# IDEA-Research/MP-Former

Measured on AMD Instinct MI355X. Metric: training images/sec COCO-instance R50 1024x1024, higher is better.
Workload: dtype bf16 (backbone, decoder) + f32 (pixel decoder, losses), as the reference's AMP; 1 GPU; COCO-instance R50, 100 queries, 80 classes, 1024x1024: full train step = R50 backbone + MSDeformAttn pixel decoder (6 layers) + MP masked decoder (9 layers, NUM_DN 1) + Hungarian matching + 60 losses + backward + grad all-reduce + clip + AdamW; head_only_workload=False, global_batch=2, per_gpu_batch=2, parallelism=dp1, msda_offsets=init, full=False, autograd_threads=backward on the launch thread, miopen_find_db=shipped

## Files before the change

mp_former_amd/csrc/gemm3_nt2.h:

```cpp
constexpr int kN2T = 512;
constexpr int kN2Kc = 256 * 16;
constexpr int kN2Op = 2 * 4 * kN2Kc;
constexpr int kN2Stage = 2 * kN2Op;
constexpr int kN2Lds = 2 * kN2Stage;

struct AccN2 {
    f32x16 v[4][2];
    __device__ __forceinline__ void zero()
    {
#pragma unroll
        for (int i = 0; i < 4; ++i)
#pragma unroll
            for (int j = 0; j < 2; ++j)
#pragma unroll
                for (int e = 0; e < 16; ++e) v[i][j][e] = 0.f;
    }
    __device__ __forceinline__ void step(const unsigned char* st, int a_base, int b_base, int lane)
    {
        const int r32 = lane & 31, gh = lane >> 5;
#pragma unroll
        for (int kh = 0; kh < 2; ++kh) {
            const int kc = 2 * kh + gh;
            const int sw = (r32 ^ (2 * kc)) * 16;
            f16x8 fb[2][2];
#pragma unroll
            for (int pl = 0; pl < 2; ++pl)
#pragma unroll
                for (int t = 0; t < 2; ++t) fb[pl][t] = as_fragh(*reinterpret_cast<const uint4*>(st + kN2Op + b_base + (pl * 4 + kc) * kN2Kc + t * 512 + sw));
#pragma unroll
            for (int i = 0; i < 4; ++i) {
                const f16x8 fah = as_fragh(*reinterpret_cast<const uint4*>(st + a_base + (0 * 4 + kc) * kN2Kc + i * 512 + sw));
                const f16x8 fal = as_fragh(*reinterpret_cast<const uint4*>(st + a_base + (1 * 4 + kc) * kN2Kc + i * 512 + sw));
#pragma unroll
                for (int j = 0; j < 2; ++j) v[i][j] = __builtin_amdgcn_mfma_f32_32x32x16_f16(fb[1][j], fah, v[i][j], 0, 0, 0);
#pragma unroll
                for (int j = 0; j < 2; ++j) v[i][j] = __builtin_amdgcn_mfma_f32_32x32x16_f16(fb[0][j], fal, v[i][j], 0, 0, 0);
#pragma unroll
                for (int j = 0; j < 2; ++j) v[i][j] = __builtin_amdgcn_mfma_f32_32x32x16_f16(fb[0][j], fah, v[i][j], 0, 0, 0);
            }
        }
    }
};

template <bool CV>
__device__ __forceinline__ void gemm3_nt2_tile(const G3N& p, const int tile, unsigned char* lds)
{
    float sc_a, sc_b, inv_a, inv_b;
    h2_scale(amax_read(p.a_amax), &sc_a, &inv_a);
    h2_scale(amax_read(p.b_amax), &sc_b, &inv_b);
    const int tn = tile % p.tiles_n, tm = (tile / p.tiles_n) % p.tiles_m, sp = tile / (p.tiles_n * p.tiles_m);
    const int m0 = tm * 256, n0 = tn * 256;
    const int r_begin = sp * p.rows_per_split, r_end = min(p.R, r_begin + p.rows_per_split);
    const int tid = threadIdx.x, lane = tid & 63, wave = tid >> 6;
    const int wr = wave >> 2, wc = wave & 3;

    const int col = tid & 255, kc0 = __builtin_amdgcn_readfirstlane(tid >> 8);
    const __amdgpu_buffer_rsrc_t ars = __builtin_amdgcn_make_buffer_rsrc(const_cast<float*>(p.a), 0, p.a_bytes, 0x00020000);
    const __amdgpu_buffer_rsrc_t brs = __builtin_amdgcn_make_buffer_rsrc(const_cast<float*>(p.b), 0, p.b_bytes, 0x00020000);
    const int acolb = (m0 + col) * 4, bcolb = (CV ? (n0 % p.cv_cin) + col : n0 + col) * 4;
    const int ldab = (int)p.lda * 4, ldbb = (int)p.ldb * 4;
    int cv_dy = 0, cv_dx = 0, cv_sh = 0, cvx0 = 0, cvy0 = 0, cvx1 = 0, cvy1 = 0;
    if constexpr (CV) {
        const int tap = n0 / p.cv_cin;
        cv_dy = tap / 3 - 1; cv_dx = tap % 3 - 1;
        cv_sh = cv_dy * p.cv_W + cv_dx;
        const int rb0 = r_begin + kc0 * 8, rb1 = rb0 + 16;
        cvx0 = rb0 % p.cv_W; cvy0 = (rb0 / p.cv_W) % p.cv_H;
        cvx1 = rb1 % p.cv_W; cvy1 = (rb1 / p.cv_W) % p.cv_H;
    }
    (void)cv_dy; (void)cv_dx; (void)cv_sh;
    float xa0[8], xa1[8], xb0[8], xb1[8];
    float csa = 0.f;
    const bool want_csa = p.csum_a && tn == 0;

#define N2_LOAD_A(r0, TAIL)                                                                                      \
    {                                                                                                            \
        _Pragma("unroll") for (int j = 0; j < 8; ++j) {                                                          \
            const int q0 = (r0) + kc0 * 8 + j, q1 = q0 + 16;                                                     \
            const int c0 = TAIL ? min(q0, r_end - 1) : q0, c1 = TAIL ? min(q1, r_end - 1) : q1;                  \
            float va0 = __int_as_float(__builtin_amdgcn_raw_buffer_load_b32(ars, acolb, c0 * ldab, 0));          \
            float va1 = __int_as_float(__builtin_amdgcn_raw_buffer_load_b32(ars, acolb, c1 * ldab, 0));          \
            if (TAIL) { va0 = q0 < r_end ? va0 : 0.f; va1 = q1 < r_end ? va1 : 0.f; }                            \
            xa0[j] = va0; xa1[j] = va1;                                                                          \
        }                                                                                                        \
    }
#define N2_LOAD_B(r0, TAIL)                                                                                      \
    {                                                                                                            \
        _Pragma("unroll") for (int j = 0; j < 8; ++j) {                                                          \
            const int q0 = (r0) + kc0 * 8 + j, q1 = q0 + 16;                                                     \
            int c0 = TAIL ? min(q0, r_end - 1) : q0, c1 = TAIL ? min(q1, r_end - 1) : q1;                        \
            if constexpr (CV) { c0 = min(max(c0 + cv_sh, 0), p.R - 1); c1 = min(max(c1 + cv_sh, 0), p.R - 1); }  \
            float vb0 = __int_as_float(__builtin_amdgcn_raw_buffer_load_b32(brs, bcolb, c0 * ldbb, 0));          \
            float vb1 = __int_as_float(__builtin_amdgcn_raw_buffer_load_b32(brs, bcolb, c1 * ldbb, 0));          \
            if constexpr (CV) {                                                                                  \
                const bool ok0 = (unsigned)(cvy0 + cv_dy) < (unsigned)p.cv_H && (unsigned)(cvx0 + j + cv_dx) < (unsigned)p.cv_W; \
                const bool ok1 = (unsigned)(cvy1 + cv_dy) < (unsigned)p.cv_H && (unsigned)(cvx1 + j + cv_dx) < (unsigned)p.cv_W; \
                vb0 = ok0 ? vb0 : 0.f; vb1 = ok1 ? vb1 : 0.f;                                                    \
            }                                                                                                    \
            if (TAIL) { vb0 = q0 < r_end ? vb0 : 0.f; vb1 = q1 < r_end ? vb1 : 0.f; }                            \
            xb0[j] = vb0; xb1[j] = vb1;                                                                          \
        }                                                                                                        \
        if constexpr (CV) {                                              \
            cvx0 += kBK; while (cvx0 >= p.cv_W) { cvx0 -= p.cv_W; cvy0 = cvy0 + 1 == p.cv_H ? 0 : cvy0 + 1; }    \
            cvx1 += kBK; while (cvx1 >= p.cv_W) { cvx1 -= p.cv_W; cvy1 = cvy1 + 1 == p.cv_H ? 0 : cvy1 + 1; }    \
        }                                                                                                        \
    }
#define N2_LOAD(r0, TAIL) { N2_LOAD_A(r0, TAIL) N2_LOAD_B(r0, TAIL) }

    AccN2 acc;
    acc.zero();
    const int a_base = wr * 128 * 16, b_base = wc * 64 * 16;
    const int sl0 = (col ^ (2 * kc0)) * 16, sl1 = (col ^ (2 * kc0 + 4)) * 16;

    if (r_begin + kBK <= r_end) N2_LOAD(r_begin, false) else N2_LOAD(r_begin, true);
    int s = 0;
    for (int r0 = r_begin; r0 < r_end; r0 += kBK, s ^= 1) {
        unsigned char* st = lds + s * kN2Stage;
        uint4 h, l;
        const bool full_next = r0 + 2 * kBK <= r_end, some_next = r0 + kBK < r_end;
        split8h(make_float4(xa0[0], xa0[1], xa0[2], xa0[3]), make_float4(xa0[4], xa0[5], xa0[6], xa0[7]), sc_a, &h, &l);
        *reinterpret_cast<uint4*>(st + (0 * 4 + kc0) * kN2Kc + sl0) = h;
        *reinterpret_cast<uint4*>(st + (1 * 4 + kc0) * kN2Kc + sl0) = l;
        split8h(make_float4(xa1[0], xa1[1], xa1[2], xa1[3]), make_float4(xa1[4], xa1[5], xa1[6], xa1[7]), sc_a, &h, &l);
        *reinterpret_cast<uint4*>(st + (0 * 4 + kc0 + 2) * kN2Kc + sl1) = h;
        *reinterpret_cast<uint4*>(st + (1 * 4 + kc0 + 2) * kN2Kc + sl1) = l;
        if (want_csa) {
#pragma unroll
            for (int j = 0; j < 8; ++j) csa += xa0[j] + xa1[j];
        }
        if (full_next) N2_LOAD_A(r0 + kBK, false) else if (some_next) N2_LOAD_A(r0 + kBK, true);
        split8h(make_float4(xb0[0], xb0[1], xb0[2], xb0[3]), make_float4(xb0[4], xb0[5], xb0[6], xb0[7]), sc_b, &h, &l);
        *reinterpret_cast<uint4*>(st + kN2Op + (0 * 4 + kc0) * kN2Kc + sl0) = h;
        *reinterpret_cast<uint4*>(st + kN2Op + (1 * 4 + kc0) * kN2Kc + sl0) = l;
        split8h(make_float4(xb1[0], xb1[1], xb1[2], xb1[3]), make_float4(xb1[4], xb1[5], xb1[6], xb1[7]), sc_b, &h, &l);
        *reinterpret_cast<uint4*>(st + kN2Op + (0 * 4 + kc0 + 2) * kN2Kc + sl1) = h;
        *reinterpret_cast<uint4*>(st + kN2Op + (1 * 4 + kc0 + 2) * kN2Kc + sl1) = l;
        if (full_next) N2_LOAD_B(r0 + kBK, false) else if (some_next) N2_LOAD_B(r0 + kBK, true);
        ws_barrier();
        acc.step(st, a_base, b_base, lane);
    }
#undef N2_LOAD
#undef N2_LOAD_A
#undef N2_LOAD_B

    float* cp = p.c + (int64_t)sp * p.c_ss;
    {
        const int r32 = lane & 31, gh = lane >> 5;
#pragma unroll
        for (int j = 0; j < 2; ++j)
#pragma unroll
            for (int i = 0; i < 4; ++i)
#pragma unroll
                for (int q = 0; q < 4; ++q) {
                    const int m = m0 + wr * 128 + i * 32 + r32, n = n0 + wc * 64 + j * 32 + 8 * q + 4 * gh;
                    float4 o = make_float4(acc.v[i][j][4 * q], acc.v[i][j][4 * q + 1], acc.v[i][j][4 * q + 2], acc.v[i][j][4 * q + 3]);
                    o = make_float4(o.x * inv_a * inv_b, o.y * inv_a * inv_b, o.z * inv_a * inv_b, o.w * inv_a * inv_b);
                    *reinterpret_cast<float4*>(cp + (int64_t)m * p.Ndim + n) = o;
                }
    }
    if (want_csa) {
        __syncthreads();
        float* red = reinterpret_cast<float*>(lds);
        if (tid < 256) red[tid] = csa;
        __syncthreads();
        if (tid >= 256) red[col] += csa;
        __syncthreads();
        if (tid < 256) p.csum_a[(int64_t)sp * p.csa_ss + m0 + tid] = red[tid];
    }
}

__global__ __launch_bounds__(kN2T, 2) void gemm3_nt2_group_kernel(G3NG g)
{
    extern __shared__ __attribute__((aligned(16))) unsigned char n2_lds[];
    const int per_xcd = (g.ntiles + 7) >> 3;
    const int tile = ((int)blockIdx.x & 7) * per_xcd + ((int)blockIdx.x >> 3);
    if (tile >= g.ntiles) return;
    int i = 0;
    while (i + 1 < g.n_items && tile >= g.tile_end[i]) ++i;
    const int first = i ? g.tile_end[i - 1] : 0;
    gemm3_nt2_tile<false>(g.it[i], tile - first, n2_lds);
}

__global__ __launch_bounds__(kN2T, 2) void gemm3_nt2_conv_kernel(G3N p)
{
    extern __shared__ __attribute__((aligned(16))) unsigned char n2_lds[];
    const int per_xcd = (p.ntiles + 7) >> 3;
    const int tile = ((int)blockIdx.x & 7) * per_xcd + ((int)blockIdx.x >> 3);
    if (tile >= p.ntiles) return;
    gemm3_nt2_tile<true>(p, tile, n2_lds);
}
```

Before: 87.42 images/sec.

## Software-pipeline the split-f16 GEMM main loop by interleaving MFMAs with staging and loads

Restructures the gemm3_nt2 main loop into a prologue plus a steady-state body. Each MFMA pair is interleaved with fine-grained split-to-f16 conversion, LDS stores into the next buffer and global loads for the stage after that, with one barrier per iteration. The A/B fragments are prefetched from LDS ahead of their MFMAs, and the conv-mode bounds check becomes a bitmask that is applied later. The goal is to hide global-load and conversion latency behind tensor-core work. It adds register pressure and more complex control flow, and sched_barriers pin the instruction order.

Result: no change. 86.97 images/sec (-0.5%).

```diff
diff --git a/mp_former_amd/csrc/gemm3_nt2.h b/mp_former_amd/csrc/gemm3_nt2.h
--- a/mp_former_amd/csrc/gemm3_nt2.h
+++ b/mp_former_amd/csrc/gemm3_nt2.h
@@ -4,6 +4,17 @@
 constexpr int kN2Stage = 2 * kN2Op;
 constexpr int kN2Lds = 2 * kN2Stage;
 
+__device__ __forceinline__ void split2h(const float x0, const float x1, const float scale, unsigned* h, unsigned* l)
+{
+    const float s0 = x0 * scale, s1 = x1 * scale;
+    const f16x2 hh = {(_Float16)s0, (_Float16)s1};
+    const float r0 = s0 - (float)hh[0], r1 = s1 - (float)hh[1];
+    const f16x2 ll = {(_Float16)r0, (_Float16)r1};
+    union { f16x2 f; unsigned u; } ch, cl;
+    ch.f = hh; cl.f = ll;
+    *h = ch.u; *l = cl.u;
+}
+
 struct AccN2 {
     f32x16 v[4][2];
     __device__ __forceinline__ void zero()
@@ -15,28 +26,39 @@
 #pragma unroll
                 for (int e = 0; e < 16; ++e) v[i][j][e] = 0.f;
     }
+    static __device__ __forceinline__ int frag_off(int lane, int kh, int pl)
+    {
+        const int kc = 2 * kh + (lane >> 5);
+        return (pl * 4 + kc) * kN2Kc + ((lane & 31) ^ (2 * kc)) * 16;
+    }
+    static __device__ __forceinline__ f16x8 frag_b(const unsigned char* st, int b_base, int lane, int kh, int pl, int t)
+    {
+        return as_fragh(*reinterpret_cast<const uint4*>(st + kN2Op + b_base + frag_off(lane, kh, pl) + t * 512));
+    }
+    static __device__ __forceinline__ f16x8 frag_a(const unsigned char* st, int a_base, int lane, int kh, int pl, int i)
+    {
+        return as_fragh(*reinterpret_cast<const uint4*>(st + a_base + frag_off(lane, kh, pl) + i * 512));
+    }
+    __device__ __forceinline__ void pair(int i, const f16x8 (&fb)[2], const f16x8& fa)
+    {
+#pragma unroll
+        for (int j = 0; j < 2; ++j) v[i][j] = __builtin_amdgcn_mfma_f32_32x32x16_f16(fb[j], fa, v[i][j], 0, 0, 0);
+    }
     __device__ __forceinline__ void step(const unsigned char* st, int a_base, int b_base, int lane)
     {
-        const int r32 = lane & 31, gh = lane >> 5;
 #pragma unroll
         for (int kh = 0; kh < 2; ++kh) {
-            const int kc = 2 * kh + gh;
-            const int sw = (r32 ^ (2 * kc)) * 16;
             f16x8 fb[2][2];
 #pragma unroll
             for (int pl = 0; pl < 2; ++pl)
 #pragma unroll
-                for (int t = 0; t < 2; ++t) fb[pl][t] = as_fragh(*reinterpret_cast<const uint4*>(st + kN2Op + b_base + (pl * 4 + kc) * kN2Kc + t * 512 + sw));
+                for (int t = 0; t < 2; ++t) fb[pl][t] = frag_b(st, b_base, lane, kh, pl, t);
 #pragma unroll
             for (int i = 0; i < 4; ++i) {
-                const f16x8 fah = as_fragh(*reinterpret_cast<const uint4*>(st + a_base + (0 * 4 + kc) * kN2Kc + i * 512 + sw));
-                const f16x8 fal = as_fragh(*reinterpret_cast<const uint4*>(st + a_base + (1 * 4 + kc) * kN2Kc + i * 512 + sw));
-#pragma unroll
-                for (int j = 0; j < 2; ++j) v[i][j] = __builtin_amdgcn_mfma_f32_32x32x16_f16(fb[1][j], fah, v[i][j], 0, 0, 0);
-#pragma unroll
-                for (int j = 0; j < 2; ++j) v[i][j] = __builtin_amdgcn_mfma_f32_32x32x16_f16(fb[0][j], fal, v[i][j], 0, 0, 0);
-#pragma unroll
-                for (int j = 0; j < 2; ++j) v[i][j] = __builtin_amdgcn_mfma_f32_32x32x16_f16(fb[0][j], fah, v[i][j], 0, 0, 0);
+                const f16x8 fah = frag_a(st, a_base, lane, kh, 0, i), fal = frag_a(st, a_base, lane, kh, 1, i);
+                pair(i, fb[1], fah);
+                pair(i, fb[0], fal);
+                pair(i, fb[0], fah);
             }
         }
     }
@@ -59,7 +81,7 @@
     const __amdgpu_buffer_rsrc_t brs = __builtin_amdgcn_make_buffer_rsrc(const_cast<float*>(p.b), 0, p.b_bytes, 0x00020000);
     const int acolb = (m0 + col) * 4, bcolb = (CV ? (n0 % p.cv_cin) + col : n0 + col) * 4;
     const int ldab = (int)p.lda * 4, ldbb = (int)p.ldb * 4;
-    int cv_dy = 0, cv_dx = 0, cv_sh = 0, cvx0 = 0, cvy0 = 0, cvx1 = 0, cvy1 = 0;
+    int cv_dy = 0, cv_dx = 0, cv_sh = 0, cvx0 = 0, cvy0 = 0, cvx1 = 0, cvy1 = 0, cv_sx = 0, cv_sy = 0;
     if constexpr (CV) {
         const int tap = n0 / p.cv_cin;
         cv_dy = tap / 3 - 1; cv_dx = tap % 3 - 1;
@@ -67,79 +89,148 @@
         const int rb0 = r_begin + kc0 * 8, rb1 = rb0 + 16;
         cvx0 = rb0 % p.cv_W; cvy0 = (rb0 / p.cv_W) % p.cv_H;
         cvx1 = rb1 % p.cv_W; cvy1 = (rb1 / p.cv_W) % p.cv_H;
-    }
-    (void)cv_dy; (void)cv_dx; (void)cv_sh;
+        cv_sx = kBK % p.cv_W; cv_sy = (kBK / p.cv_W) % p.cv_H;
+    }
+    (void)cv_dy; (void)cv_dx; (void)cv_sh; (void)cv_sx; (void)cv_sy;
     float xa0[8], xa1[8], xb0[8], xb1[8];
     float csa = 0.f;
+    unsigned cv_ok = 0;
+    (void)cv_ok;
     const bool want_csa = p.csum_a && tn == 0;
 
-#define N2_LOAD_A(r0, TAIL)                                                                                      \
-    {                                                                                                            \
-        _Pragma("unroll") for (int j = 0; j < 8; ++j) {                                                          \
-            const int q0 = (r0) + kc0 * 8 + j, q1 = q0 + 16;                                                     \
-            const int c0 = TAIL ? min(q0, r_end - 1) : q0, c1 = TAIL ? min(q1, r_end - 1) : q1;                  \
-            float va0 = __int_as_float(__builtin_amdgcn_raw_buffer_load_b32(ars, acolb, c0 * ldab, 0));          \
-            float va1 = __int_as_float(__builtin_amdgcn_raw_buffer_load_b32(ars, acolb, c1 * ldab, 0));          \
-            if (TAIL) { va0 = q0 < r_end ? va0 : 0.f; va1 = q1 < r_end ? va1 : 0.f; }                            \
-            xa0[j] = va0; xa1[j] = va1;                                                                          \
-        }                                                                                                        \
-    }
-#define N2_LOAD_B(r0, TAIL)                                                                                      \
-    {                                                                                                            \
-        _Pragma("unroll") for (int j = 0; j < 8; ++j) {                                                          \
-            const int q0 = (r0) + kc0 * 8 + j, q1 = q0 + 16;                                                     \
-            int c0 = TAIL ? min(q0, r_end - 1) : q0, c1 = TAIL ? min(q1, r_end - 1) : q1;                        \
-            if constexpr (CV) { c0 = min(max(c0 + cv_sh, 0), p.R - 1); c1 = min(max(c1 + cv_sh, 0), p.R - 1); }  \
-            float vb0 = __int_as_float(__builtin_amdgcn_raw_buffer_load_b32(brs, bcolb, c0 * ldbb, 0));          \
-            float vb1 = __int_as_float(__builtin_amdgcn_raw_buffer_load_b32(brs, bcolb, c1 * ldbb, 0));          \
-            if constexpr (CV) {                                                                                  \
-                const bool ok0 = (unsigned)(cvy0 + cv_dy) < (unsigned)p.cv_H && (unsigned)(cvx0 + j + cv_dx) < (unsigned)p.cv_W; \
-                const bool ok1 = (unsigned)(cvy1 + cv_dy) < (unsigned)p.cv_H && (unsigned)(cvx1 + j + cv_dx) < (unsigned)p.cv_W; \
-                vb0 = ok0 ? vb0 : 0.f; vb1 = ok1 ? vb1 : 0.f;                                                    \
+#define N2_LOAD_A(r0, TAIL, j)                                                                                   \
+    {                                                                                                            \
+        const int q0 = (r0) + kc0 * 8 + (j), q1 = q0 + 16;                                                       \
+        const int c0 = TAIL ? min(q0, r_end - 1) : q0, c1 = TAIL ? min(q1, r_end - 1) : q1;                      \
+        float va0 = __int_as_float(__builtin_amdgcn_raw_buffer_load_b32(ars, acolb, c0 * ldab, 0));              \
+        float va1 = __int_as_float(__builtin_amdgcn_raw_buffer_load_b32(ars, acolb, c1 * ldab, 0));              \
+        if (TAIL) { va0 = q0 < r_end ? va0 : 0.f; va1 = q1 < r_end ? va1 : 0.f; }                                \
+        xa0[j] = va0; xa1[j] = va1;                                                                              \
+    }
+#define N2_LOAD_B(r0, TAIL, j)                                                                                   \
+    {                                                                                                            \
+        const int q0 = (r0) + kc0 * 8 + (j), q1 = q0 + 16;                                                       \
+        int c0 = TAIL ? min(q0, r_end - 1) : q0, c1 = TAIL ? min(q1, r_end - 1) : q1;                            \
+        if constexpr (CV) { c0 = min(max(c0 + cv_sh, 0), p.R - 1); c1 = min(max(c1 + cv_sh, 0), p.R - 1); }      \
+        float vb0 = __int_as_float(__builtin_amdgcn_raw_buffer_load_b32(brs, bcolb, c0 * ldbb, 0));              \
+        float vb1 = __int_as_float(__builtin_amdgcn_raw_buffer_load_b32(brs, bcolb, c1 * ldbb, 0));              \
+        if constexpr (CV) {                                                                                      \
+            const bool ok0 = (unsigned)(cvy0 + cv_dy) < (unsigned)p.cv_H && (unsigned)(cvx0 + (j) + cv_dx) < (unsigned)p.cv_W; \
+            const bool ok1 = (unsigned)(cvy1 + cv_dy) < (unsigned)p.cv_H && (unsigned)(cvx1 + (j) + cv_dx) < (unsigned)p.cv_W; \
+               \
+            if ((j) == 0) cv_ok = 0;                                                                             \
+            cv_ok |= (ok0 ? 1u : 0u) << (j) | (ok1 ? 1u : 0u) << (8 + (j));                                      \
+        }                                                                                                        \
+        if (TAIL) { vb0 = q0 < r_end ? vb0 : 0.f; vb1 = q1 < r_end ? vb1 : 0.f; }                                \
+        xb0[j] = vb0; xb1[j] = vb1;                                                                              \
+        if constexpr (CV) {                                                                                      \
+            if ((j) == 7) {                                              \
+                cvx0 += cv_sx; cvy0 += cv_sy; if (cvx0 >= p.cv_W) { cvx0 -= p.cv_W; ++cvy0; } cvy0 = cvy0 >= p.cv_H ? cvy0 - p.cv_H : cvy0; \
+                cvx1 += cv_sx; cvy1 += cv_sy; if (cvx1 >= p.cv_W) { cvx1 -= p.cv_W; ++cvy1; } cvy1 = cvy1 >= p.cv_H ? cvy1 - p.cv_H : cvy1; \
             }                                                                                                    \
-            if (TAIL) { vb0 = q0 < r_end ? vb0 : 0.f; vb1 = q1 < r_end ? vb1 : 0.f; }                            \
-            xb0[j] = vb0; xb1[j] = vb1;                                                                          \
-        }                                                                                                        \
-        if constexpr (CV) {                                              \
-            cvx0 += kBK; while (cvx0 >= p.cv_W) { cvx0 -= p.cv_W; cvy0 = cvy0 + 1 == p.cv_H ? 0 : cvy0 + 1; }    \
-            cvx1 += kBK; while (cvx1 >= p.cv_W) { cvx1 -= p.cv_W; cvy1 = cvy1 + 1 == p.cv_H ? 0 : cvy1 + 1; }    \
-        }                                                                                                        \
-    }
-#define N2_LOAD(r0, TAIL) { N2_LOAD_A(r0, TAIL) N2_LOAD_B(r0, TAIL) }
+        }                                                                                                        \
+    }
 
     AccN2 acc;
     acc.zero();
     const int a_base = wr * 128 * 16, b_base = wc * 64 * 16;
     const int sl0 = (col ^ (2 * kc0)) * 16, sl1 = (col ^ (2 * kc0 + 4)) * 16;
 
-    if (r_begin + kBK <= r_end) N2_LOAD(r_begin, false) else N2_LOAD(r_begin, true);
-    int s = 0;
-    for (int r0 = r_begin; r0 < r_end; r0 += kBK, s ^= 1) {
-        unsigned char* st = lds + s * kN2Stage;
-        uint4 h, l;
-        const bool full_next = r0 + 2 * kBK <= r_end, some_next = r0 + kBK < r_end;
-        split8h(make_float4(xa0[0], xa0[1], xa0[2], xa0[3]), make_float4(xa0[4], xa0[5], xa0[6], xa0[7]), sc_a, &h, &l);
-        *reinterpret_cast<uint4*>(st + (0 * 4 + kc0) * kN2Kc + sl0) = h;
-        *reinterpret_cast<uint4*>(st + (1 * 4 + kc0) * kN2Kc + sl0) = l;
-        split8h(make_float4(xa1[0], xa1[1], xa1[2], xa1[3]), make_float4(xa1[4], xa1[5], xa1[6], xa1[7]), sc_a, &h, &l);
-        *reinterpret_cast<uint4*>(st + (0 * 4 + kc0 + 2) * kN2Kc + sl1) = h;
-        *reinterpret_cast<uint4*>(st + (1 * 4 + kc0 + 2) * kN2Kc + sl1) = l;
-        if (want_csa) {
-#pragma unroll
-            for (int j = 0; j < 8; ++j) csa += xa0[j] + xa1[j];
-        }
-        if (full_next) N2_LOAD_A(r0 + kBK, false) else if (some_next) N2_LOAD_A(r0 + kBK, true);
-        split8h(make_float4(xb0[0], xb0[1], xb0[2], xb0[3]), make_float4(xb0[4], xb0[5], xb0[6], xb0[7]), sc_b, &h, &l);
-        *reinterpret_cast<uint4*>(st + kN2Op + (0 * 4 + kc0) * kN2Kc + sl0) = h;
-        *reinterpret_cast<uint4*>(st + kN2Op + (1 * 4 + kc0) * kN2Kc + sl0) = l;
-        split8h(make_float4(xb1[0], xb1[1], xb1[2], xb1[3]), make_float4(xb1[4], xb1[5], xb1[6], xb1[7]), sc_b, &h, &l);
-        *reinterpret_cast<uint4*>(st + kN2Op + (0 * 4 + kc0 + 2) * kN2Kc + sl1) = h;
-        *reinterpret_cast<uint4*>(st + kN2Op + (1 * 4 + kc0 + 2) * kN2Kc + sl1) = l;
-        if (full_next) N2_LOAD_B(r0 + kBK, false) else if (some_next) N2_LOAD_B(r0 + kBK, true);
+    unsigned hb[4], lb[4];
+#define N2_STAGE(nx, u, LA, LB)                                                                                  \
+    {                                                                                                            \
+        if ((u) < 4) split2h(xa0[2 * ((u) & 3)], xa0[2 * ((u) & 3) + 1], sc_a, &hb[(u) & 3], &lb[(u) & 3]);      \
+        else if ((u) < 8) {                                                                                      \
+            split2h(xa1[2 * ((u) & 3)], xa1[2 * ((u) & 3) + 1], sc_a, &hb[(u) & 3], &lb[(u) & 3]);               \
+            csa += xa0[2 * ((u) & 3)] + xa1[2 * ((u) & 3)];                                                      \
+            csa += xa0[2 * ((u) & 3) + 1] + xa1[2 * ((u) & 3) + 1];                                              \
+        }                                                                                                        \
+        else if ((u) < 12) {                                                                                     \
+            if constexpr (CV) {                                                                                  \
+                xb0[2 * ((u) & 3)] = (cv_ok >> (2 * ((u) & 3))) & 1 ? xb0[2 * ((u) & 3)] : 0.f;                  \
+                xb0[2 * ((u) & 3) + 1] = (cv_ok >> (2 * ((u) & 3) + 1)) & 1 ? xb0[2 * ((u) & 3) + 1] : 0.f;      \
+            }                                                                                                    \
+            split2h(xb0[2 * ((u) & 3)], xb0[2 * ((u) & 3) + 1], sc_b, &hb[(u) & 3], &lb[(u) & 3]);               \
+        }                                                                                                        \
+        else if ((u) < 16) {                                                                                     \
+            if constexpr (CV) {                                                                                  \
+                xb1[2 * ((u) & 3)] = (cv_ok >> (8 + 2 * ((u) & 3))) & 1 ? xb1[2 * ((u) & 3)] : 0.f;              \
+                xb1[2 * ((u) & 3) + 1] = (cv_ok >> (9 + 2 * ((u) & 3))) & 1 ? xb1[2 * ((u) & 3) + 1] : 0.f;      \
+            }                                                                                                    \
+            split2h(xb1[2 * ((u) & 3)], xb1[2 * ((u) & 3) + 1], sc_b, &hb[(u) & 3], &lb[(u) & 3]);               \
+        }                                                                                                        \
+        if ((u) < 16 && ((u) & 3) == 3) {                                                                        \
+            unsigned char* dst = (nx) + ((u) >= 8 ? kN2Op : 0) + ((u) & 4 ? 2 * kN2Kc + sl1 : sl0) + kc0 * kN2Kc; \
+            *reinterpret_cast<uint4*>(dst) = make_uint4(hb[0], hb[1], hb[2], hb[3]);                             \
+            *reinterpret_cast<uint4*>(dst + 4 * kN2Kc) = make_uint4(lb[0], lb[1], lb[2], lb[3]);                 \
+        }                                                                                                        \
+        if ((u) >= 8 && (u) < 16) LA((u) - 8)                                                                    \
+        if ((u) >= 16) LB((u) - 16)                                                                              \
+    }
+#define N2_BODY(LA, LB)                                                                                          \
+    {                                                                                                            \
+        const unsigned char* st = lds + s * kN2Stage;                                                            \
+        unsigned char* nx = lds + (s ^ 1) * kN2Stage;                                                            \
+        f16x8 fbh[2][2], fbl[2], fah[2], fal;      \
+        _Pragma("unroll") for (int t = 0; t < 2; ++t) fbl[t] = AccN2::frag_b(st, b_base, lane, 0, 1, t);         \
+        _Pragma("unroll") for (int t = 0; t < 2; ++t) fbh[0][t] = AccN2::frag_b(st, b_base, lane, 0, 0, t);      \
+        fah[0] = AccN2::frag_a(st, a_base, lane, 0, 0, 0);                                                       \
+        fal = AccN2::frag_a(st, a_base, lane, 0, 1, 0);                                                          \
+        _Pragma("unroll") for (int u = 0; u < 24; ++u) {                                                         \
+            const int kh = u / 12, i = (u % 12) / 3, pr = u % 3, par = (u / 3) & 1;                              \
+                                                                                  \
+            if (pr == 0 && u + 3 < 24) fah[par ^ 1] = AccN2::frag_a(st, a_base, lane, (u + 3) / 12, 0, ((u + 3) % 12) / 3); \
+            if (pr == 2 && u + 1 < 24) fal = AccN2::frag_a(st, a_base, lane, (u + 1) / 12, 1, ((u + 1) % 12) / 3); \
+            if (u == 8) { _Pragma("unroll") for (int t = 0; t < 2; ++t) fbh[1][t] = AccN2::frag_b(st, b_base, lane, 1, 0, t); } \
+            if (u == 10) { _Pragma("unroll") for (int t = 0; t < 2; ++t) fbl[t] = AccN2::frag_b(st, b_base, lane, 1, 1, t); } \
+            if (pr == 0) acc.pair(i, fbl, fah[par]);                                                             \
+            else if (pr == 1) acc.pair(i, fbh[kh], fal);                                                         \
+            else acc.pair(i, fbh[kh], fah[par]);                                                                 \
+            N2_STAGE(nx, u, LA, LB)                                                                              \
+            __builtin_amdgcn_sched_barrier(0);                                                                   \
+        }                                                                                                        \
+        ws_barrier();                     \
+        s ^= 1;                                                                                                  \
+    }
+
+    if (r_begin + kBK <= r_end) {
+#pragma unroll
+        for (int j = 0; j < 8; ++j) N2_LOAD_A(r_begin, false, j)
+#pragma unroll
+        for (int j = 0; j < 8; ++j) N2_LOAD_B(r_begin, false, j)
+    } else {
+#pragma unroll
+        for (int j = 0; j < 8; ++j) N2_LOAD_A(r_begin, true, j)
+#pragma unroll
+        for (int j = 0; j < 8; ++j) N2_LOAD_B(r_begin, true, j)
+    }
+    int s = 0, r0 = r_begin;
+    {
+        const bool some_next = r0 + kBK < r_end;
+#define N2_LA(j) if (some_next) N2_LOAD_A(r0 + kBK, true, j)
+#define N2_LB(j) if (some_next) N2_LOAD_B(r0 + kBK, true, j)
+#pragma unroll
+        for (int u = 0; u < 24; ++u) N2_STAGE(lds, u, N2_LA, N2_LB)
+#undef N2_LA
+#undef N2_LB
         ws_barrier();
-        acc.step(st, a_base, b_base, lane);
-    }
-#undef N2_LOAD
+    }
+#define N2_LA(j) N2_LOAD_A(r0 + 2 * kBK, false, j)
+#define N2_LB(j) N2_LOAD_B(r0 + 2 * kBK, false, j)
+    for (; r0 + 3 * kBK <= r_end; r0 += kBK) N2_BODY(N2_LA, N2_LB)
+#undef N2_LA
+#undef N2_LB
+#define N2_LA(j) if (some_next) N2_LOAD_A(r0 + 2 * kBK, true, j)
+#define N2_LB(j) if (some_next) N2_LOAD_B(r0 + 2 * kBK, true, j)
+    for (; r0 + kBK < r_end; r0 += kBK) {
+        const bool some_next = r0 + 2 * kBK < r_end;
+        N2_BODY(N2_LA, N2_LB)
+    }
+#undef N2_LA
+#undef N2_LB
+    acc.step(lds + s * kN2Stage, a_base, b_base, lane);
+#undef N2_BODY
+#undef N2_STAGE
 #undef N2_LOAD_A
 #undef N2_LOAD_B
 
```
